# NUStatBioinfo/DegNorm

Hardware: AMD Instinct MI355X
Metric: genes/sec (20k genes x 10 samples, 5 iters) (higher is better)
Workload: dtype f64

## Files before the change

### degnorm_amd/csrc/dn_kernels.hpp

```cpp
#pragma once
#include <hip/hip_runtime.h>
#include <stdint.h>
#include <type_traits>
#include "dn_reduce.hpp"
#include "dn_dpp_ops.hpp"

#ifdef DN_MARKS
#define DN_MARK(name) asm volatile("; DN_MARK " name)
#else
#define DN_MARK(name)
#endif

namespace dn {

constexpr int TRACE_LEN = 48;
constexpr int MAX_BINS = 64;
constexpr int P_MAX = 64;

enum { EXIT_LOW_COV = 0, EXIT_ZERO_SAMPLE = 1, EXIT_MEDIAN = 2, EXIT_NO_LOOP = 3,
       EXIT_REFINED = 4, EXIT_REFINE_FALLBACK = 5, EXIT_NOT_FOUND_FALLBACK = 6 };
enum { LOOP_NATURAL = 0, LOOP_PERFECT = 1, LOOP_VALUE_ERROR = 2, LOOP_ZERO_ROWSUM = 3, LOOP_MIN_BINS = 4,
       LOOP_NOT_ENTERED = 5 };
enum { ST_OK = 0, ST_ARPACK = -1, ST_EMPTY_MIN = -2, ST_VALUE_ERROR = -3,
       ST_NO_CONVERGENCE = -4 };
// ... 1161 lines not shown
        if constexpr (W > 1) {
            dn_sync();
            for (int e = tid; e < NG; e += NT) {
                double tsum = sm.xw[0][e];
#pragma unroll
                for (int ww = 1; ww < W; ww++) tsum += sm.xw[ww][e];
                sm.tot[e] = tsum;
            }
        }
        dn_sync();
    };

    pass(true, 0);
    {
        const double tr = wave_allsum(lane < P ? sm.tot[lane * (lane + 1) / 2 + lane] : 0.0);
        if (!(tr > 0.0)) return ST_ARPACK;
    }
    { const int r = top_eig_rows_lds<P>(sm.tot, uv, vv, theta, maxs); steps += r; noconv = noconv || r > maxs; }
    bool cold_every_solve;
    {
        double um = lane < P ? uv[lane] : 1.0;
#pragma unroll
        for (int o = 32; o >= 1; o >>= 1) um = fmin(um, __shfl_xor(um, o));
        cold_every_solve = __builtin_amdgcn_readfirstlane((int) (um < WARM_START_MIN_COMPONENT)) != 0;
    }
#pragma clang loop unroll(disable)
    for (int t = 0; t < T; t++) {
        pass(false, t);
        int r;
        if (!cold_every_solve) r = top_eig_rows_lds<P>(sm.tot, uv, vv, theta, maxs);
        else {
            unsigned long long todo = P >= 64 ? ~0ull : ((1ull << P) - 1ull);
            double bul = 0.0, bth = -1.0;
            int sum = 0;
            bool capped = false;
            while (todo) {
                const unsigned long long comp = gram_component(sm.tot, __builtin_ctzll(todo), P);
                todo &= ~comp;
                wave_fence();
                uv[lane] = ((comp >> lane) & 1ull) ? 1.0 / sqrt((double) __builtin_popcountll(comp)) : 0.0;
                wave_fence();
                double th = 0.0;
                const int rr = top_eig_rows_lds<P>(sm.tot, uv, vv, th, maxs);
                sum += rr < maxs ? rr : maxs;
                capped = capped || rr > maxs;
                const double ul = uv[lane];
                if (th > bth) { bth = th; bul = ul; }
            }
            wave_fence();
            uv[lane] = bul;
            wave_fence();
            theta = bth > 0.0 ? bth : 0.0;
            r = capped ? maxs + 1 : (sum < maxs ? sum : maxs);
        }
        steps += r; noconv = noconv || r > maxs;
    }
    bcast_rows<P>(lane < P ? uv[lane] : 0.0, u);
    return ST_OK;
}

#ifndef DN_RT_MAX_COLS
#define DN_RT_MAX_COLS 12
#endif
#ifndef DN_RT_MAX_P
#define DN_RT_MAX_P 12
#endif
#ifndef DN_RT_MIN_P
#define DN_RT_MIN_P 2
#endif
#if defined(DN_P) && DN_P >= DN_RT_MIN_P && DN_P <= DN_RT_MAX_P
#define DN_REG_TIER 1
#define DN_KERNEL_WAVES 2
#define DN_RT_CLAIM() asm volatile("" ::: "a255")
#else
#define DN_REG_TIER 0
#define DN_KERNEL_WAVES 1
#define DN_RT_CLAIM()
#endif
#define DN_RAW_MAX_P 12
template <int P> constexpr bool raw_units() { return DN_REG_TIER != 0 && P <= DN_RAW_MAX_P && P < DN_MG_MIN_P; }

template <int IDX> __device__ __forceinline__ int agpr_get1();
template <int IDX> __device__ __forceinline__ void agpr_put1(int v);
#define DN_AGPR_ACCESSORS(N)                                                                                              \
    template <> __device__ __forceinline__ int agpr_get1<N>() { int v; asm volatile("v_accvgpr_read_b32 %0, a" #N : "=v"(v)); return v; } \
    template <> __device__ __forceinline__ void agpr_put1<N>(int v) { asm volatile("v_accvgpr_write_b32 a" #N ", %0" : : "v"(v)); }
#define DN_AGPR_REGS(X) \
    X(0) X(1) X(2) X(3) X(4) X(5) X(6) X(7) X(8) X(9) X(10) X(11) X(12) X(13) X(14) X(15) \
    X(16) X(17) X(18) X(19) X(20) X(21) X(22) X(23) X(24) X(25) X(26) X(27) X(28) X(29) X(30) X(31) \
    X(32) X(33) X(34) X(35) X(36) X(37) X(38) X(39) X(40) X(41) X(42) X(43) X(44) X(45) X(46) X(47) \
    X(48) X(49) X(50) X(51) X(52) X(53) X(54) X(55) X(56) X(57) X(58) X(59) X(60) X(61) X(62) X(63) \
    X(64) X(65) X(66) X(67) X(68) X(69) X(70) X(71) X(72) X(73) X(74) X(75) X(76) X(77) X(78) X(79) \
    X(80) X(81) X(82) X(83) X(84) X(85) X(86) X(87) X(88) X(89) X(90) X(91) X(92) X(93) X(94) X(95) \
    X(96) X(97) X(98) X(99) X(100) X(101) X(102) X(103) X(104) X(105) X(106) X(107) X(108) X(109) X(110) X(111) \
    X(112) X(113) X(114) X(115) X(116) X(117) X(118) X(119) X(120) X(121) X(122) X(123) X(124) X(125) X(126) X(127) \
    X(128) X(129) X(130) X(131) X(132) X(133) X(134) X(135) X(136) X(137) X(138) X(139) X(140) X(141) X(142) X(143) \
    X(144) X(145) X(146) X(147) X(148) X(149) X(150) X(151) X(152) X(153) X(154) X(155) X(156) X(157) X(158) X(159) \
    X(160) X(161) X(162) X(163) X(164) X(165) X(166) X(167) X(168) X(169) X(170) X(171) X(172) X(173) X(174) X(175) \
    X(176) X(177) X(178) X(179) X(180) X(181) X(182) X(183) X(184) X(185) X(186) X(187) X(188) X(189) X(190) X(191) \
    X(192) X(193) X(194) X(195) X(196) X(197) X(198) X(199) X(200) X(201) X(202) X(203) X(204) X(205) X(206) X(207) \
    X(208) X(209) X(210) X(211) X(212) X(213) X(214) X(215) X(216) X(217) X(218) X(219) X(220) X(221) X(222) X(223) \
    X(224) X(225) X(226) X(227) X(228) X(229) X(230) X(231) X(232) X(233) X(234) X(235) X(236) X(237) X(238) X(239) \
    X(240) X(241) X(242) X(243) X(244) X(245) X(246) X(247) X(248) X(249) X(250) X(251) X(252) X(253) X(254) X(255)
DN_AGPR_REGS(DN_AGPR_ACCESSORS)
#undef DN_AGPR_ACCESSORS
#undef DN_AGPR_REGS
template <int IDX> __device__ __forceinline__ double agpr_get()
{
    const int lo = agpr_get1<IDX>(), hi = agpr_get1<IDX + 1>();
    return __hiloint2double(hi, lo);
}
template <int IDX> __device__ __forceinline__ void agpr_put(double v)
{
    agpr_put1<IDX>(__double2loint(v));
    agpr_put1<IDX + 1>(__double2hiint(v));
}

template <int P, int BASE> __device__ __forceinline__ void rt_read(double (&a)[P])
{
    static_for<0, P>([&](auto ic) { constexpr int I = decltype(ic)::value; a[I] = agpr_get<BASE + 2 * I>(); });
}
template <int P, int BASE> __device__ __forceinline__ void rt_write(const double (&a)[P])
{
    static_for<0, P>([&](auto ic) { constexpr int I = decltype(ic)::value; agpr_put<BASE + 2 * I>(a[I]); });
}
template <int P, int BASE> __device__ __forceinline__ void rt_read_counts(double (&xd)[P])
{
    static_for<0, (P + 1) / 2>([&](auto jc) {
        constexpr int J = decltype(jc)::value;
        const unsigned w = (unsigned) agpr_get1<BASE + J>();
        xd[2 * J] = (double) (w & 0xffffu);
        if constexpr (2 * J + 1 < P) xd[2 * J + 1] = (double) (w >> 16);
    });
}
template <int P, int BASE> __device__ __forceinline__ void rt_write_counts(const float (&x)[P])
{
    static_for<0, (P + 1) / 2>([&](auto jc) {
        constexpr int J = decltype(jc)::value;
        unsigned w = (unsigned) x[2 * J];
        if constexpr (2 * J + 1 < P) w |= ((unsigned) x[2 * J + 1]) << 16;
        agpr_put1<BASE + J>((int) w);
    });
}
template <int P, bool X16> constexpr int rt_col_regs() { return 2 * P + (X16 ? (P + 1) / 2 : 0); }
template <int P, bool X16> constexpr int rt_cols()
{
    return (P >= DN_RT_MIN_P && P <= DN_RT_MAX_P) ? (256 / rt_col_regs<P, X16>() < DN_RT_MAX_COLS ? 256 / rt_col_regs<P, X16>() : DN_RT_MAX_COLS) : 0;
}
template <int P> constexpr int rt_regs_used()
{
    return rt_cols<P, true>() * rt_col_regs<P, true>() > rt_cols<P, false>() * rt_col_regs<P, false>()
               ? rt_cols<P, true>() * rt_col_regs<P, true>() : rt_cols<P, false>() * rt_col_regs<P, false>();
}
constexpr int RT_BATCH = 48;
#define DN_RT_SAVE_IDX(r) ((size_t) (r) * NT + DN_TIDX)
template <int N, int NT> __device__ __forceinline__ void rt_save(int *save, int need)
{
    static_for<0, (N + RT_BATCH - 1) / RT_BATCH>([&](auto bc) {
        constexpr int B = decltype(bc)::value * RT_BATCH;
        constexpr int CNT = (N - B) < RT_BATCH ? (N - B) : RT_BATCH;
        if (B < need) {
            int v[CNT];
            static_for<0, CNT>([&](auto ic) { constexpr int I = decltype(ic)::value; v[I] = agpr_get1<B + I>(); });
#pragma unroll
            for (int i = 0; i < CNT; i++) save[DN_RT_SAVE_IDX(B + i)] = v[i];
            asm volatile("" ::: "memory");
        }
    });
}
template <int N, int NT> __device__ __forceinline__ void rt_restore(const int *save, int need)
{
    static_for<0, (N + RT_BATCH - 1) / RT_BATCH>([&](auto bc) {
        constexpr int B = decltype(bc)::value * RT_BATCH;
        constexpr int CNT = (N - B) < RT_BATCH ? (N - B) : RT_BATCH;
        if (B < need) {
            int v[CNT];
#pragma unroll
            for (int i = 0; i < CNT; i++) v[i] = save[DN_RT_SAVE_IDX(B + i)];
            static_for<0, CNT>([&](auto ic) { constexpr int I = decltype(ic)::value; agpr_put1<B + I>(v[I]); });
            asm volatile("" ::: "memory");
        }
    });
}
template <int P, int NT> constexpr size_t rt_save_bytes() { return (size_t) rt_regs_used<P>() * 4 * NT; }

template <int P, int NT, bool X16, bool FULL = false, bool ONCHIP = false, bool SAFE = false>
__device__ __forceinline__ void nmf_body(const float *Fb_, double *Lg_, double *rs_, double *sv_,
                                         int n, int S, int nL, int T, int first_i)
{
    Smem<P, NT> &sm = g_sm;
    double *lam = g_lam + (DN_UNITS > 1 ? (size_t) DN_UNIT * (size_t) nL * (P + (P & 1)) : 0);
    gF_cptr Fb = (gF_cptr) uniform_ptr(Fb_);
    gdouble_ptr Lg = (gdouble_ptr) uniform_ptr(Lg_);
    gdouble_ptr rs = (gdouble_ptr) uniform_ptr(rs_);
    gdouble_ptr sv = (gdouble_ptr) uniform_ptr(sv_);
    n = __builtin_amdgcn_readfirstlane(n);
    S = __builtin_amdgcn_readfirstlane(S);
    nL = __builtin_amdgcn_readfirstlane(nL);
    T = __builtin_amdgcn_readfirstlane(T);
    const bool first = __builtin_amdgcn_readfirstlane(first_i) != 0;
    double inv[P], u[P], theta = 0.0;
    int steps = 0;
    const int maxs = __builtin_amdgcn_readfirstlane(g_gs.max_steps);
    bool noconv = false;
#pragma unroll
    for (int i = 0; i < P; i++) inv[i] = uniform(g_gs.inv[i]);
    long long stamp[4] = {0, 0, 0, 0};
#ifdef DN_STAMP
#define DN_T0() const long long t0_ = __builtin_amdgcn_s_memtime()
#define DN_T1(slot) stamp[slot] += __builtin_amdgcn_s_memtime() - t0_
#else
#define DN_T0()
#define DN_T1(slot) (void) stamp
#endif
    constexpr int NG = P * (P + 1) / 2;
    constexpr int CH_MAX = P <= 15 ? 120 : 90;
    constexpr int SW = (NG + CH_MAX - 1) / CH_MAX;
    constexpr int CH = (NG + SW - 1) / SW;
    constexpr int PS = P + (P & 1);
    const int tid = DN_TIDX;
    constexpr int RT = DN_REG_TIER ? rt_cols<P, X16>() : 0;
    constexpr int CS = rt_col_regs<P, X16>();
    constexpr int NR = RT * NT;
    constexpr bool RAW = raw_units<P>();
    double ud[P], ur[P];
    const int nLe = (n < NR + nL) ? n : NR + nL;
    const int kS0 = NR + nL;
    if constexpr (P >= DN_MG_MIN_P) {
        const int st = mg_core<P, NT>(Fb, Lg, lam, n, nL, T, u, theta, steps, maxs, noconv);
        if (st != ST_OK) { if (tid == 0) g_gs.status = st; dn_sync(); return; }
    } else {
    gram_t G[CH];

#ifdef DN_STAMP
    const long long t_cold0 = __builtin_amdgcn_s_memtime();
#endif
#pragma unroll
    for (int i = 0; i < CH; i++) G[i] = 0.0;
    {
        float xq[P];
        if (tid < n) load_x<P>(Fb, tid, xq);
#pragma clang loop unroll(disable)
        for (int k = tid; k < n; k += NT) {
            double f[P];
#pragma unroll
            for (int i = 0; i < P; i++) f[i] = (double) xq[i] * inv[i];
            load_x<P>(Fb, k + NT < n ? k + NT : k, xq);
            gram_add_range<P, 0, CH>(G, f);
        }
    }
    block_sum_lds<CH, P, NT, gram_t>(G, sm);
    static_for<1, SW>([&](auto qc) {
        constexpr int Q = decltype(qc)::value;
        constexpr int NQ = (NG - Q * CH) < CH ? (NG - Q * CH) : CH;
        gram_t Gq[NQ];
#pragma unroll
        for (int i = 0; i < NQ; i++) Gq[i] = 0.0;
#pragma clang loop unroll(disable)
        for (int k = tid; k < n; k += NT) {
            double f[P];
            load_f<P>(Fb, k, inv, f);
            gram_add_range<P, Q * CH, NQ>(Gq, f);
        }
        block_sum_lds<NQ, P, NT, gram_t, false, Q * CH>(Gq, g_sm);
    });
    {
        double tr = 0.0;
#pragma unroll
        for (int i = 0; i < P; i++) tr += sm.tot[i * (i + 1) / 2 + i];
        if (!(tr > 0.0)) { if (tid == 0) g_gs.status = ST_ARPACK; dn_sync(); return; }
    }
    Solver<P> solver;
    {
        double tr = 0.0;
#pragma unroll
        for (int i = 0; i < P; i++) tr += sm.tot[i * (i + 1) / 2 + i];
        solver.cold(tr, u);
    }
    {
        const int r = SAFE ? solve_by_blocks<P>(solver, sm.tot, Smem<P, NT>::ZSLOT, u, theta, maxs)
                           : solver.run(sm.tot, Smem<P, NT>::ZSLOT, u, theta, T == 0, maxs, true);
        steps += r; noconv = noconv || r > maxs;
    }
    const double c = 1.0 / sqrt((double) T);
    auto pass_u = [&]() {
        if constexpr (RAW) {
            const int k = Solver<P>::row_of_lane() < P ? Solver<P>::row_of_lane() : P - 1;
            const double vt = solver.iterate_of_row() * g_gs.inv[k], vh = solver.iterate_of_row() * g_gs.scl[k];
#pragma unroll
            for (int i = 0; i < P; i++) { ud[i] = Solver<P>::bcast_component(vt, i); ur[i] = Solver<P>::bcast_component(vh, i); }
        } else {
#pragma unroll
            for (int i = 0; i < P; i++) { u[i] = uniform(u[i]); ud[i] = u[i]; ur[i] = u[i]; }
        }
    };
    pass_u();

    static_for<0, RT>([&](auto rc) {
        constexpr int R = decltype(rc)::value;
        const int k = tid + R * NT;
        if (k < n) {
            float xf[P];
            double f[P];
            load_x<P>(Fb, k, xf);
            pass_counts<P, RAW>(xf, inv, f);
            rt_write<P, CS * R>(f);
            if constexpr (X16) rt_write_counts<P, CS * R + 2 * P>(xf);
        }
    });
    for (int k = NR + tid; k < nLe; k += NT) {
        double f[P], a[PS];
        { float xf[P]; load_x<P>(Fb, k, xf); pass_counts<P, RAW>(xf, inv, f); }
#pragma unroll
        for (int i = 0; i < PS; i++) a[i] = i < P ? f[i] : 0.0;
        lds_col_write<PS>(lam + (size_t) (k - NR) * PS, a);
    }
    if constexpr (!ONCHIP) {
        for (int k = kS0 + tid; k < n; k += NT) {
            double f[P];
            { float xf[P]; load_x<P>(Fb, k, xf); pass_counts<P, RAW>(xf, inv, f); }
            spill_col_write<P>(spill_col<P>(Lg, k), f);
        }
    }
#ifdef DN_STAMP
    stamp[3] += __builtin_amdgcn_s_memtime() - t_cold0;
#endif
    constexpr bool G0 = FULL && ONCHIP && SW == 1;
    constexpr bool SQ = Solver<P>::SQUARE && SW == 1 && !SAFE;
#pragma clang loop unroll(disable)
    for (int t = 0; t < T; t++) {
        DN_MARK("iter_begin");
        if constexpr (!G0) {
#pragma unroll
            for (int i = 0; i < CH; i++) G[i] = 0.0;
        }
        DN_MARK("zeroed");
        { DN_T0();
        const int dir = (t & 1) ? -1 : 1;

        auto reg_tier = [&]() {
            if constexpr (RT > 0 && X16) {
                auto column = [&](auto rc) {
                    constexpr int R = decltype(rc)::value;
                    double f[P], a[P];
                    rt_read_counts<P, CS * R + 2 * P>(f);
                    if constexpr (!RAW) {
#pragma unroll
                        for (int i = 0; i < P; i++) f[i] *= inv[i];
                    }
                    rt_read<P, CS * R>(a);
                    col_update<P>(f, a, ud, ur, c);
                    if constexpr (G0 && R == 0) gram_set_range<P, 0, CH>(G, a); else gram_add_range<P, 0, CH>(G, a);
                    rt_write<P, CS * R>(a);
                };
                if constexpr (FULL) {
                    static_for<0, RT>([&](auto rc) { column(rc); __builtin_amdgcn_sched_barrier(0); });
                } else {
                    static_for<0, RT>([&](auto rc) {
                        constexpr int R = decltype(rc)::value;
                        if (tid + R * NT < n) column(rc);
                    });
                }
            } else if constexpr (RT > 0) {
                float xq[P];
                if (tid < n) load_x<P>(Fb, tid, xq);
                static_for<0, RT>([&](auto rc) {
                    constexpr int R = decltype(rc)::value;
                    const int k = tid + R * NT;
                    if (k < n) {
                        double f[P], a[P];
                        pass_counts<P, RAW>(xq, inv, f);
                        if constexpr (R + 1 < RT) load_x<P>(Fb, k + NT < n ? k + NT : k, xq);
                        rt_read<P, CS * R>(a);
                        col_update<P>(f, a, ud, ur, c);
                        gram_add_range<P, 0, CH>(G, a);
                        rt_write<P, CS * R>(a);
                    }
                });
            }
        };
        auto lds_tier = [&]() {
            const int first = NR + tid;
            const int cnt = first < nLe ? (nLe - first + NT - 1) / NT : 0;
            const int step = dir * NT;
            int k = dir > 0 ? first : first + (cnt - 1) * NT;
            float xq[P];
            if (cnt > 0) load_x<P>(Fb, k, xq);
#pragma clang loop unroll(disable)
            for (int j = 0; j < cnt; j++, k += step) {
                double f[P], a[PS];
                lds_col_read<PS>(lam + (size_t) (k - NR) * PS, a);
                pass_counts<P, RAW>(xq, inv, f);
                load_x<P>(Fb, j + 1 < cnt ? k + step : k, xq);
                double aa[P];
#pragma unroll
                for (int i = 0; i < P; i++) aa[i] = a[i];
                col_update<P>(f, aa, ud, ur, c);
                gram_add_range<P, 0, CH>(G, aa);
#pragma unroll
                for (int i = 0; i < P; i++) a[i] = aa[i];
                lds_col_write<PS>(lam + (size_t) (k - NR) * PS, a);
            }
        };
        auto spill_tier = [&]() {
            if constexpr (ONCHIP) return;
            int tq = tid;
            asm volatile("" : "+v"(tq));
            const int first = kS0 + tq;
            if (first >= n) return;
            const int step = dir * NT;
            const int last = first + (n - 1 - first) / NT * NT;
            int k = dir > 0 ? first : last;
            const int kend = dir > 0 ? last : first;
            float xn[P];
            double an[P];
            load_x<P>(Fb, k, xn);
            spill_col_read<P>(spill_col<P>(Lg, k), an);
            bool more;
#pragma clang loop unroll(disable)
            do {
                double f[P], a[P];
                pass_counts<P, RAW>(xn, inv, f);
#pragma unroll
                for (int i = 0; i < P; i++) a[i] = an[i];
                const int kn = dir > 0 ? min(k + step, kend) : max(k + step, kend);
                load_x<P>(Fb, kn, xn);
                spill_col_read<P>(spill_col<P>(Lg, kn), an);
                col_update<P>(f, a, ud, ur, c);
                gram_add_range<P, 0, CH>(G, a);
                spill_col_write<P>(spill_col<P>(Lg, k), a);
                more = k != kend;
                k += step;
            } while (more);
        };
#if defined(DN_STAMP) && defined(DN_EXP_TIER)
#define DN_TIER(id, call) do { if (DN_EXP_TIER == id) { const long long tt_ = __builtin_amdgcn_s_memtime(); call; stamp[0] += __builtin_amdgcn_s_memtime() - tt_; } else { call; } } while (0)
#else
#define DN_TIER(id, call) call
#endif
        if constexpr (G0) { DN_MARK("reg_tier"); DN_TIER(1, reg_tier()); DN_MARK("lds_tier"); DN_TIER(2, lds_tier()); }
        else if (dir > 0) { DN_MARK("reg_tier"); DN_TIER(1, reg_tier()); DN_MARK("lds_tier"); DN_TIER(2, lds_tier()); DN_MARK("spill_tier"); DN_TIER(3, spill_tier()); }
        else { DN_MARK("spill_tier_b"); DN_TIER(3, spill_tier()); DN_MARK("lds_tier_b"); DN_TIER(2, lds_tier()); DN_MARK("reg_tier_b"); DN_TIER(1, reg_tier()); }
        DN_MARK("pass_end");
#if !(defined(DN_STAMP) && defined(DN_EXP_TIER))
        DN_T1(0);
#endif
        }
        { DN_T0(); block_sum_lds<CH, P, NT, gram_t, Solver<P>::SHIFTED, 0, RAW, SQ>(G, sm, solver.shift(), solver.scale(), t & 1); DN_T1(1); }
        DN_MARK("reduced");
        static_for<1, SW>([&](auto qc) {
            constexpr int Q = decltype(qc)::value;
            constexpr int NQ = (NG - Q * CH) < CH ? (NG - Q * CH) : CH;
            gram_t Gq[NQ];
#pragma unroll
            for (int i = 0; i < NQ; i++) Gq[i] = 0.0;
            static_assert(SW == 1 || RT == 0, "the later sweeps do not read the register tier");
#pragma clang loop unroll(disable)
            for (int k = NR + tid; k < nLe; k += NT) {
                double a[PS], aa[P];
                lds_col_read<PS>(lam + (size_t) (k - NR) * PS, a);
#pragma unroll
                for (int i = 0; i < P; i++) aa[i] = a[i];
                gram_add_range<P, Q * CH, NQ>(Gq, aa);
            }
#pragma clang loop unroll(disable)
            for (int k = kS0 + tid; k < n; k += NT) {
                double aa[P];
                spill_col_read<P>(spill_col<P>(Lg, k), aa);
                gram_add_range<P, Q * CH, NQ>(Gq, aa);
            }
            block_sum_lds<NQ, P, NT, gram_t, Solver<P>::SHIFTED, Q * CH>(Gq, g_sm, solver.shift());
        });
        { DN_T0();
        double u_unused[P];
        double (&us_)[P] = RAW ? u_unused : u;
        const int r = SAFE ? solve_by_blocks<P>(solver, sm.tot, Smem<P, NT>::ZSLOT, us_, theta, maxs)
                           : solver.template run<SQ>(sm.tot, Smem<P, NT>::ZSLOT, us_, theta, t == T - 1, maxs, false,
                                                     sm.sq + wave_id() * Smem<P, NT>::SQ_LEN);
        steps += r; noconv = noconv || r > maxs;
        pass_u();
        DN_MARK("solved");
        DN_T1(2);
        }
    }
    if constexpr (SQ && NT > 64) dn_sync();
    if constexpr (RAW) {
#pragma unroll
        for (int i = 0; i < P; i++) u[i] = Solver<P>::bcast_component(solver.iterate_of_row(), i);
    }
    }

#ifdef DN_STAMP
    const long long t_fin0 = __builtin_amdgcn_s_memtime();
#endif
    double invf[P];
#pragma unroll
    for (int i = 0; i < P; i++) invf[i] = RAW ? uniform(g_gs.inv[i]) : inv[i];
    double acc[2 * P + 1];
#pragma unroll
    for (int i = 0; i < 2 * P + 1; i++) acc[i] = 0.0;
    auto fin = [&](int k, const double (&f)[P], const double (&l_)[P]) {
        double s, r, l0[P];
#pragma unroll
        for (int i = 0; i < P; i++) l0[i] = RAW ? l_[i] * invf[i] : l_[i];
        col_final<P>(f, l0, u, first, acc, s, r);
        rs[k] = r;
        if (first) sv[k] = s;
    };
    static_for<0, RT>([&](auto rc) {
        constexpr int R = decltype(rc)::value;
        const int k = tid + R * NT;
        if (k < n) {
            double f[P], l[P];
            if constexpr (X16) {
                rt_read_counts<P, CS * R + 2 * P>(f);
#pragma unroll
                for (int i = 0; i < P; i++) f[i] *= invf[i];
            } else load_f<P>(Fb, k, invf, f);
            rt_read<P, CS * R>(l);
            fin(k, f, l);
        }
    });
    float xqf[P];
    if (NR + tid < n) load_x<P>(Fb, NR + tid, xqf);
#pragma clang loop unroll(disable)
    for (int k = NR + tid; k < n; k += NT) {
        double f[P], l[P];
#pragma unroll
        for (int i = 0; i < P; i++) f[i] = (double) xqf[i] * invf[i];
        load_x<P>(Fb, k + NT < n ? k + NT : k, xqf);
        if (k < nLe) {
            double al[PS];
            lds_col_read<PS>(lam + (size_t) (k - NR) * PS, al);
#pragma unroll
            for (int i = 0; i < P; i++) l[i] = al[i];
        } else spill_col_read<P>(spill_col<P>(Lg, k), l);
        fin(k, f, l);
    }
    block_sum_lds<2 * P + 1, P, NT, double>(acc, sm);
    for (int e = tid; e < 2 * P + 1; e += NT) g_gs.sums[e] = sm.tot[e];
    if (tid == 0) {
#pragma unroll
        for (int i = 0; i < P; i++) g_gs.u[i] = u[i];
        g_gs.theta = theta;
        g_gs.steps += steps;
        g_gs.status = noconv ? ST_NO_CONVERGENCE : ST_OK;
#ifdef DN_STAMP
        g_gs.stamp[0] += stamp[0]; g_gs.stamp[1] += stamp[1]; g_gs.stamp[2] += stamp[2];
        g_gs.stamp[4] += __builtin_amdgcn_s_memtime() - t_fin0; g_gs.stamp[5] += stamp[3];
#endif
    }
    dn_sync();
}

template <int P, int NT, bool SAFE = false>
__device__ __attribute__((noinline)) void nmf_call(const float *Fb_, double *Lg_, double *rs_, double *sv_, double *rtsave_,
                                                   int n, int S, int nL, int T, int first_i, int x16_i)
{
    constexpr int NSAVE = DN_REG_TIER ? rt_regs_used<P>() : 0;
    int *rtsave = reinterpret_cast<int *>(uniform_ptr(rtsave_));
#ifdef DN_STAMP
    const long long t_call0 = __builtin_amdgcn_s_memtime();
#endif
    const int n_u = __builtin_amdgcn_readfirstlane(n);
    const int need = DN_REG_TIER ? ((n_u + NT - 1) / NT) * rt_col_regs<P, true>() : 0;
    rt_save<NSAVE, NT>(rtsave, need);
    if constexpr (SAFE) {
        nmf_body<P, NT, false, false, false, true>(Fb_, Lg_, rs_, sv_, n, S, nL, T, first_i);
    } else if (DN_REG_TIER && __builtin_amdgcn_readfirstlane(x16_i) != 0) {
        constexpr bool X = DN_REG_TIER != 0;
        const int nL_u = __builtin_amdgcn_readfirstlane(nL);
        if (X && n_u >= rt_cols<P, X>() * NT && n_u <= rt_cols<P, X>() * NT + nL_u)
            nmf_body<P, NT, X, X, X>(Fb_, Lg_, rs_, sv_, n, S, nL, T, first_i);
        else if (X && n_u >= rt_cols<P, X>() * NT) nmf_body<P, NT, X, X>(Fb_, Lg_, rs_, sv_, n, S, nL, T, first_i);
        else nmf_body<P, NT, X, false>(Fb_, Lg_, rs_, sv_, n, S, nL, T, first_i);
    } else nmf_body<P, NT, false>(Fb_, Lg_, rs_, sv_, n, S, nL, T, first_i);
    rt_restore<NSAVE, NT>(rtsave, need);
#ifdef DN_STAMP
    if (DN_TIDX == 0) g_gs.stamp[3] += __builtin_amdgcn_s_memtime() - t_call0;
#endif
}


template <int P> __device__ __forceinline__ double lds_max(const double *v)
{ double m = v[0];
#pragma unroll
  for (int i = 1; i < P; i++) { const double t = v[i]; m = t > m ? t : m; } return m; }
template <int P> __device__ __forceinline__ double lds_min(const double *v)
{ double m = v[0];
#pragma unroll
  for (int i = 1; i < P; i++) { const double t = v[i]; m = t < m ? t : m; } return m; }

template <int P, int NT>
__global__ __launch_bounds__(NT * DN_UNITS, DN_KERNEL_WAVES) void k_baseline(IterArgs A)
{
    constexpr int W = NT / 64;
    Smem<P, NT> &sm = g_sm;
    GeneState<P> &gs = g_gs;
    const int tid = DN_TIDX, lane = lane_id(), w = wave_id();
    const int S = A.S;
    const int nL = A.lds_cols;
    char *slot = A.ws + ((size_t) blockIdx.x * DN_UNITS + DN_UNIT) * A.slot_bytes;
    float *Fs = reinterpret_cast<float *>(slot);
    float *Fb = Fs + (size_t) P * S;
    double *Lg = reinterpret_cast<double *>(Fb + (size_t) P * S);
    double *sv = Lg + (size_t) (P + (P & 1)) * S;
    double *rs = sv + S;
    double *rtsave = rs + 2 * (size_t) S;
    DN_RT_CLAIM();
    if (tid < P) { gs.inv[tid] = A.inv_scale[tid]; gs.scl[tid] = 1.0 / A.inv_scale[tid]; }
    if (tid == 0) gs.max_steps = A.max_steps > 0 ? A.max_steps : EIG_MAX_STEPS_DEFAULT;
    if constexpr (P <= 16) { for (int t = tid; t < W * Smem<P, NT>::SQ_LEN; t += NT) sm.sq[t] = 0.0; }
    for (int t = tid; t < Smem<P, NT>::NX; t += NT) {
        bool diag = false;
        int ra = 0, rb = 0;
#pragma unroll
        for (int i = 0; i < P; i++) {
            diag = diag || (t == i * (i + 1) / 2 + i);
            if (t >= i * (i + 1) / 2) { ra = i; rb = t - i * (i + 1) / 2; }
        }
        if constexpr (P <= 16) sm.sqi[t] = (t < P * (P + 1) / 2) ? (ra * Smem<P, NT>::SQ_STR + rb) | ((rb * Smem<P, NT>::SQ_STR + ra) << 16) : 0;
        if constexpr (raw_units<P>())
            sm.dsel[t] = (t < P * (P + 1) / 2) ? (diag ? -1.0 : 1.0) * A.inv_scale[ra] * A.inv_scale[rb < P ? rb : 0] : 0.0;
        else sm.dsel[t] = diag ? 1.0 : 0.0;
        if (t == Smem<P, NT>::ZSLOT) sm.tot[t] = 0.0;
    }

    for (;;) {
        if (tid == 0) sm.gene = atomicAdd(A.counter, 1);
        dn_sync();
        const int q = sm.gene;
        dn_sync();
        if (q >= A.n_genes) break;
        const int g = A.order[q];
        const int L = A.glen[g];
        const float *x = A.cov + A.goff[g];

        int n0 = 0, n_calls = 0, n_drops = 0, exit_code = EXIT_LOW_COV, loop_reason = LOOP_NOT_ENTERED;
        int status = ST_OK, flag = 0, emode = EM_INPUT;
        long long sum_cols = 0;
#ifdef DN_STAMP
        const long long t_gene0 = __builtin_amdgcn_s_memtime();
        long long t_ret = 0, t_book = 0;
#endif
        int32_t *tr = A.trace + (size_t) g * TRACE_LEN;
        if (tid < P) { gs.rho[tid] = 0.0; gs.K[tid] = 0.0; gs.us[tid] = 0.0; }
        if (tid == 0) { gs.steps = 0; gs.stamp[0] = gs.stamp[1] = gs.stamp[2] = gs.stamp[3] = gs.stamp[4] = gs.stamp[5] = 0; }

        double thr;
        int x16;
        {
            const float *rmx = A.rowmax + (size_t) g * P;
            double gmax = (double) rmx[0] / A.scale[0];
#pragma unroll
            for (int i = 1; i < P; i++) { const double v = (double) rmx[i] / A.scale[i]; gmax = v > gmax ? v : gmax; }
            thr = 0.1 * gmax;
            x16 = A.x16[g];
        }

        const int rate = A.rate;
        const long long ds0 = (rate > 1 && A.ds_start) ? A.ds_start[g] : -1;
        const int M = ds0 >= 0 ? (ds0 < L ? (int) ((L - 1 - ds0) / rate) + 1 : 0) : L;
        const int seg = ((M + W - 1) / W + 63) & ~63;
        const int jb = w * seg, je = (jb + seg < M) ? jb + seg : M;

        {
            double sumF[P];
#pragma unroll
            for (int i = 0; i < P; i++) sumF[i] = 0.0;
            int base = 0;
            for (int pass = 0; pass < 2; pass++) {
                int run = 0;
                for (int c = jb; c < je; c += 64) {
                    const int m = c + lane;
                    bool hi = false;
                    float xv[P];
                    double f[P];
                    if (m < je) {
                        const long long j = ds0 >= 0 ? ds0 + (long long) m * rate : (long long) m;
                        double cm = 0.0;
#pragma unroll
                        for (int i = 0; i < P; i++) { xv[i] = x[(size_t) i * L + j]; f[i] = (double) xv[i] / A.scale[i]; cm = f[i] > cm ? f[i] : cm; }
                        hi = cm > thr;
                    }
                    const unsigned long long mask = __ballot(hi);
                    if (pass == 1 && hi) {
                        const int pos = base + run + __popcll(mask & ((1ull << lane) - 1ull));
#pragma unroll
                        for (int i = 0; i < P; i++) {
                            Fs[(size_t) i * S + pos] = xv[i];
                            Fb[(size_t) pos * P + i] = xv[i];
                            sumF[i] += f[i];
                        }
                    }
                    run += __popcll(mask);
                }
                if (pass == 0) {
                    if (lane == 0) sm.cnt[w] = run;
                    dn_sync();
                    n0 = 0;
#pragma unroll
                    for (int ww = 0; ww < W; ww++) { if (ww < w) base += sm.cnt[ww]; n0 += sm.cnt[ww]; }
                    dn_sync();
                    if (n0 < A.min_hc) break;
                }
            }
            if (n0 >= A.min_hc) {
                block_sum<P, P, NT>(sumF, sm);
                if (tid == 0) {
#pragma unroll
                    for (int i = 0; i < P; i++) gs.sumF[i] = sumF[i];
                }
            }
            dn_sync();
        }

#ifdef DN_STAMP
        const long long t_scan1 = __builtin_amdgcn_s_memtime();
#endif
        int n = n0;
        if (n0 >= A.min_hc) {
            if (!(lds_min<P>(gs.sumF) > 0.0)) exit_code = EXIT_ZERO_SAMPLE;
            else {
                const double min_gene_len = fmax(2.0, ceil(200.0 * (1.0 / (double) rate)));
                const double min_bins = ceil((double) A.bins * 0.2);
                int csize = 1, n_bins = 0;
                bool first = true, in_loop = false;
                for (;;) {
#ifdef DN_STAMP
                    if (t_ret != 0) t_book += __builtin_amdgcn_s_memtime() - t_ret;
#endif
                    nmf_call<P, NT>(Fb, Lg, rs, sv, rtsave, n, S, nL, A.T, first ? 1 : 0, x16);
                    if constexpr (P < DN_MG_MIN_P) {
                        const int st_call = __builtin_amdgcn_readfirstlane(gs.status);
                        bool unsafe = st_call == ST_NO_CONVERGENCE;
                        if (st_call == ST_OK) {
#pragma unroll
                            for (int i = 0; i < P; i++)
                                unsafe = unsafe || (gs.u[i] < WARM_START_MIN_COMPONENT && gs.sums[1 + P + i] > 0.0);
                        }
                        if (__builtin_amdgcn_readfirstlane((int) unsafe) != 0) {
                            dn_sync();
                            nmf_call<P, NT, true>(Fb, Lg, rs, sv, rtsave, n, S, nL, A.T, first ? 1 : 0, x16);
                        }
                    }
#ifdef DN_STAMP
                    t_ret = __builtin_amdgcn_s_memtime();
#endif
                    if (gs.status != ST_OK) { status = gs.status; break; }
                    const double *u = gs.u, *sums = gs.sums;
                    const double theta = gs.theta;
                    n_calls++; sum_cols += n;
                    if (first) {
                        if (tid == 0) {
                            const double sig = sqrt(theta);
                            gs.sig0 = sig;
#pragma unroll
                            for (int i = 0; i < P; i++) {
                                gs.us[i] = u[i];
                                gs.K[i] = u[i] * sig;
                                gs.rho[i] = 1.0 - sums[1 + P + i] / (u[i] * sums[0] + 1.0);
                                gs.rho_fb[i] = 1.0 - gs.sumF[i] / (sums[1 + i] + 1.0);
                            }
                        }
                        dn_sync();
                        double med;
                        {
                            double om[P];
#pragma unroll
                            for (int i = 0; i < P; i++) om[i] = 1.0 - gs.rho[i];
                            med = median_of<P>(om);
                        }
                        if (med > 1.0) { exit_code = EXIT_MEDIAN; break; }
                        emode = (n0 < L) ? EM_EXPAND : EM_RAW;
                        exit_code = EXIT_NO_LOOP;
                        if (!((double) n0 >= min_gene_len && lds_min<P>(gs.rho) <= 0.2 && !A.skip)) break;
                        in_loop = true;
                        csize = (n0 + A.bins - 1) / A.bins;
                        n_bins = (n0 + csize - 1) / csize;
                        if (tid < n_bins) sm.alive[tid] = tid;
                        dn_sync();
                        first = false;
                    } else {
                        bool zero_row = false;
#pragma unroll
                        for (int i = 0; i < P; i++) zero_row = zero_row || (sums[1 + P + i] == 0.0);
                        if (tid == 0) {
                            const double sg = sqrt(theta);
#pragma unroll
                            for (int i = 0; i < P; i++) {
                                gs.K[i] = u[i] * sg;
                                if (!zero_row) gs.rho[i] = 1.0 - sums[1 + P + i] / (sums[1 + i] + 1.0);
                            }
                        }
                        dn_sync();
                        if (zero_row) { loop_reason = LOOP_ZERO_ROWSUM; break; }
                        if ((double) n_bins <= min_bins || (double) n < min_gene_len) { loop_reason = LOOP_MIN_BINS; break; }
                    }
                    if (!(lds_max<P>(gs.rho) > 0.1)) break;
                    flag = 1;
                    loop_reason = LOOP_NATURAL;
                    for (int b = w; b < n_bins; b += W) {
                        const int kb = b * csize, ke = (kb + csize < n) ? kb + csize : n;
                        double part = 0.0;
                        for (int k = kb + lane; k < ke; k += 4 * 64) {
                            double v[4];
#pragma unroll
                            for (int c = 0; c < 4; c++) v[c] = (k + 64 * c < ke) ? rs[k + 64 * c] : 0.0;
#pragma unroll
                            for (int c = 0; c < 4; c++) if (k + 64 * c < ke) part += v[c];
                        }
                        part = wave_sum1(part);
                        if (lane == 0) sm.ss[b] = part / (double) (ke - kb);
                    }
                    dn_sync();
                    double best = -INFINITY; int drop = 0;
                    for (int b = 0; b < n_bins; b++) { const double v = sm.ss[b]; if (v > best) { best = v; drop = b; } }
                    dn_sync();
                    if (best == 0.0) { loop_reason = LOOP_PERFECT; break; }
                    const int kb = drop * csize;
                    const int dlen = ((kb + csize < n) ? kb + csize : n) - kb;
                    if (tid == 0) {
                        for (int b = drop; b < n_bins - 1; b++) sm.alive[b] = sm.alive[b + 1];
                        if (n_drops < 32) tr[8 + n_drops] = drop;
                    }
                    n_bins--;
                    n -= dlen;
                    n_drops++;
                    dn_sync();
                    for (int k0 = kb + tid; k0 < n; k0 += 4 * NT) {
                        float v[4][P];
#pragma unroll
                        for (int c = 0; c < 4; c++) {
                            const int k = (k0 + c * NT < n) ? k0 + c * NT : k0;
                            const int a = k / csize;
                            const int ko = sm.alive[a] * csize + (k - a * csize);
#pragma unroll
                            for (int i = 0; i < P; i++) v[c][i] = Fs[(size_t) i * S + ko];
                        }
#pragma unroll
                        for (int c = 0; c < 4; c++) {
                            if (k0 + c * NT < n) {
#pragma unroll
                                for (int i = 0; i < P; i++) Fb[(size_t) (k0 + c * NT) * P + i] = v[c][i];
                            }
                        }
                    }
                    dn_sync();
                    if (n < 2) { loop_reason = LOOP_VALUE_ERROR; break; }
                }

                if (in_loop && status == ST_OK) {
                    bool fallback = false;
                    if (lds_max<P>(gs.rho) < 0.2) {
                        double K[P];
#pragma unroll
                        for (int i = 0; i < P; i++) K[i] = gs.K[i];
                        status = fix_k<P>(K);
                        if (status == ST_OK) {
                            double se[1] = {0.0};
                            for (int k = tid; k < n0; k += NT) {
                                double m = -INFINITY;
#pragma unroll
                                for (int i = 0; i < P; i++) {
                                    const double qv = ((double) Fs[(size_t) i * S + k] * gs.inv[i]) / K[i];
                                    m = qv > m ? qv : m;
                                }
                                se[0] += m;
                            }
                            block_sum<1, P, NT>(se, sm);
                            double rmax = -INFINITY;
#pragma unroll
                            for (int i = 0; i < P; i++) {
                                const double r = 1.0 - gs.sumF[i] / (K[i] * se[0] + 1.0);
                                rmax = r > rmax ? r : rmax;
                            }
                            dn_sync();
                            if (rmax > 0.9) { fallback = true; exit_code = EXIT_REFINE_FALLBACK; }
                            else {
                                exit_code = EXIT_REFINED; emode = (n0 < L) ? EM_EXPAND : EM_REFINED;
                                if (tid == 0) {
#pragma unroll
                                    for (int i = 0; i < P; i++) { gs.K[i] = K[i]; gs.rho[i] = 1.0 - gs.sumF[i] / (K[i] * se[0] + 1.0); }
                                }
                            }
                        }
                    } else { fallback = true; exit_code = EXIT_NOT_FOUND_FALLBACK; }
                    if (fallback && status == ST_OK) {
                        if (tid == 0) {
#pragma unroll
                            for (int i = 0; i < P; i++) { gs.K[i] = gs.us[i] * gs.sig0; gs.rho[i] = gs.rho_fb[i]; }
                        }
                        emode = (n0 < L) ? EM_EXPAND : EM_CLAMPED;
                    }
                    dn_sync();
                }
                if (status == ST_OK && exit_code >= EXIT_NO_LOOP && n0 < L) {
                    double K[P];
#pragma unroll
                    for (int i = 0; i < P; i++) K[i] = gs.K[i];
                    status = fix_k<P>(K);
                    dn_sync();
                    if (tid == 0) {
#pragma unroll
                        for (int i = 0; i < P; i++) gs.K[i] = K[i];
                    }
                }
            }
        }
        dn_sync();

        const bool zero_out = (status != ST_OK) || exit_code <= EXIT_MEDIAN;
        if (zero_out) { emode = EM_INPUT; if (status != ST_OK) flag = 0; }

        if (tid == 0) {
#pragma unroll
            for (int i = 0; i < P; i++) {
                A.rho[(size_t) g * P + i] = zero_out ? 0.0 : gs.rho[i];
                A.kfin[(size_t) g * P + i] = (emode == EM_CLAMPED || emode == EM_RAW) ? gs.us[i] : gs.K[i];
            }
            A.flags[g] = flag;
            A.emode[g] = emode;
            tr[0] = n0; tr[1] = n_calls; tr[2] = (int32_t) sum_cols; tr[3] = exit_code; tr[4] = loop_reason;
            tr[5] = n_drops; tr[6] = status; tr[7] = gs.steps;
#ifdef DN_STAMP
            tr[40] = (int32_t) (gs.stamp[0] >> 10); tr[41] = (int32_t) (gs.stamp[1] >> 10); tr[42] = (int32_t) (gs.stamp[2] >> 10);
            tr[44] = (int32_t) (gs.stamp[3] >> 10); tr[45] = (int32_t) (gs.stamp[4] >> 10); tr[46] = (int32_t) (gs.stamp[5] >> 10);
            tr[43] = (int32_t) ((__builtin_amdgcn_s_memtime() - t_gene0) >> 10);
            tr[47] = (int32_t) ((t_scan1 - t_gene0) >> 10);
            tr[39] = (int32_t) (t_book >> 10);
            tr[38] = (int32_t) ((t_ret != 0 ? __builtin_amdgcn_s_memtime() - t_ret : 0) >> 10);
#endif
        }
        if (A.want_est && (emode == EM_CLAMPED || emode == EM_RAW)) {
            double *dst = A.svec + A.svoff[g];
            for (int k = tid; k < n0; k += NT) dst[k] = sv[k];
        }
        dn_sync();
    }
}

template <int P, int NT>
__global__ __launch_bounds__(NT) void k_ratio_svd(InitArgs A)
{
    constexpr int NG = P * (P + 1) / 2;
    Smem<P, NT> &sm = g_sm;
    const int tid = DN_TIDX;
    for (;;) {
        if (tid == 0) sm.gene = atomicAdd(A.counter, 1);
        dn_sync();
        const int q = sm.gene;
        dn_sync();
        if (q >= A.n_genes) break;
        const int g = A.order[q];
        const int L = A.glen[g];
        const float *x = A.cov + A.goff[g];
        int status = ST_OK;
        double acc[2 * P];
#pragma unroll
        for (int i = 0; i < 2 * P; i++) acc[i] = 0.0;
        if (L < 2) status = ST_VALUE_ERROR;
        else {
            double G[NG];
#pragma unroll
            for (int i = 0; i < NG; i++) G[i] = 0.0;
            for (int j = tid; j < L; j += NT) {
// ... 112 lines not shown
```

Before: 15440.

## Software-pipeline LDS tier loop two columns per iteration with prefetched reads

Rewrites the LDS-resident column loop to handle two columns per iteration. The next column's LDS read is issued before the current column's Gram accumulation and write-back, so LDS latency can overlap with compute. Scheduling barriers pin the interleaving. Separately, the non-convergence flag is packed into a high bit of the step counter to save a register. Risks include higher register pressure and subtle edge handling for odd counts and direction.

Result: no change. 15500 (median of 6 runs) (+0.4%).

```diff
diff --git a/degnorm_amd/csrc/dn_kernels.hpp b/degnorm_amd/csrc/dn_kernels.hpp
--- a/degnorm_amd/csrc/dn_kernels.hpp
+++ b/degnorm_amd/csrc/dn_kernels.hpp
@@ -1388,6 +1388,7 @@
     int steps = 0;
     const int maxs = __builtin_amdgcn_readfirstlane(g_gs.max_steps);
     bool noconv = false;
+    constexpr int NOCONV_BIT = 1 << 30;
 #pragma unroll
     for (int i = 0; i < P; i++) inv[i] = uniform(g_gs.inv[i]);
     long long stamp[4] = {0, 0, 0, 0};
@@ -1465,7 +1466,7 @@
     {
         const int r = SAFE ? solve_by_blocks<P>(solver, sm.tot, Smem<P, NT>::ZSLOT, u, theta, maxs)
                            : solver.run(sm.tot, Smem<P, NT>::ZSLOT, u, theta, T == 0, maxs, true);
-        steps += r; noconv = noconv || r > maxs;
+        steps = (steps + r) | (r > maxs ? NOCONV_BIT : 0);
     }
     const double c = 1.0 / sqrt((double) T);
     auto pass_u = [&]() {
@@ -1565,27 +1566,72 @@
             }
         };
         auto lds_tier = [&]() {
-            const int first = NR + tid;
-            const int cnt = first < nLe ? (nLe - first + NT - 1) / NT : 0;
+            int tq;
+            asm volatile("v_mov_b32 %0, %1" : "=v"(tq) : "v"(tid));
+            const int first = NR + tq;
+            if (first >= nLe) return;
             const int step = dir * NT;
-            int k = dir > 0 ? first : first + (cnt - 1) * NT;
+            const int last = first + (nLe - 1 - first) / NT * NT;
+            int k = dir > 0 ? first : last;
+            const int kend = dir > 0 ? last : first;
+            double *const pend = lam + (size_t) (kend - NR) * PS;
+            auto next_k = [&](int kk) {
+                if constexpr (G0) return kk != kend ? kk + step : kk;
+                else return dir > 0 ? min(kk + step, kend) : max(kk + step, kend);
+            };
+            auto next_p = [&](double *pp, int kk) {
+                double *const pn = pp + step * PS;
+                if constexpr (G0) return kk != kend ? pn : pp;
+                else return dir > 0 ? (pn < pend ? pn : pend) : (pn > pend ? pn : pend);
+            };
+            double *pa = lam + (size_t) (k - NR) * PS;
             float xq[P];
-            if (cnt > 0) load_x<P>(Fb, k, xq);
+            double a1[PS];
+            load_x<P>(Fb, k, xq);
+            lds_col_read<PS>(pa, a1);
+            bool more;
 #pragma clang loop unroll(disable)
-            for (int j = 0; j < cnt; j++, k += step) {
-                double f[P], a[PS];
-                lds_col_read<PS>(lam + (size_t) (k - NR) * PS, a);
-                pass_counts<P, RAW>(xq, inv, f);
-                load_x<P>(Fb, j + 1 < cnt ? k + step : k, xq);
-                double aa[P];
-#pragma unroll
-                for (int i = 0; i < P; i++) aa[i] = a[i];
-                col_update<P>(f, aa, ud, ur, c);
+            do {
+                double f1[P], a2[PS], aa[P];
+                pass_counts<P, RAW>(xq, inv, f1);
+                const int k0 = k;
+                const int kb = next_k(k);
+                double *const pb = next_p(pa, k);
+                load_x<P>(Fb, kb, xq);
+#pragma unroll
+                for (int i = 0; i < P; i++) aa[i] = a1[i];
+                col_update<P>(f1, aa, ud, ur, c);
+                __builtin_amdgcn_sched_barrier(0);
+                lds_col_read<PS>(pb, a2);
+                __builtin_amdgcn_sched_barrier(0);
                 gram_add_range<P, 0, CH>(G, aa);
-#pragma unroll
-                for (int i = 0; i < P; i++) a[i] = aa[i];
-                lds_col_write<PS>(lam + (size_t) (k - NR) * PS, a);
-            }
+                __builtin_amdgcn_sched_barrier(0);
+#pragma unroll
+                for (int i = 0; i < P; i++) a1[i] = aa[i];
+                lds_col_write<PS>(pa, a1);
+                __builtin_amdgcn_sched_barrier(0);
+                double f2[P], bb[P];
+                pass_counts<P, RAW>(xq, inv, f2);
+                more = kb != kend;
+                k = next_k(kb);
+                pa = next_p(pb, kb);
+                load_x<P>(Fb, k, xq);
+#pragma unroll
+                for (int i = 0; i < P; i++) bb[i] = a2[i];
+                col_update<P>(f2, bb, ud, ur, c);
+#pragma unroll
+                for (int i = 0; i < P; i++) asm volatile("" : "+v"(bb[i]));
+                __builtin_amdgcn_sched_barrier(0);
+                lds_col_read<PS>(pa, a1);
+                __builtin_amdgcn_sched_barrier(0);
+                if (k0 != kend) {
+                    gram_add_range<P, 0, CH>(G, bb);
+                    __builtin_amdgcn_sched_barrier(0);
+#pragma unroll
+                    for (int i = 0; i < P; i++) a2[i] = bb[i];
+                    lds_col_write<PS>(pb, a2);
+                }
+            } while (more);
         };
         auto spill_tier = [&]() {
             if constexpr (ONCHIP) return;
@@ -1662,12 +1708,14 @@
         const int r = SAFE ? solve_by_blocks<P>(solver, sm.tot, Smem<P, NT>::ZSLOT, us_, theta, maxs)
                            : solver.template run<SQ>(sm.tot, Smem<P, NT>::ZSLOT, us_, theta, t == T - 1, maxs, false,
                                                      sm.sq + wave_id() * Smem<P, NT>::SQ_LEN);
-        steps += r; noconv = noconv || r > maxs;
+        steps = (steps + r) | (r > maxs ? NOCONV_BIT : 0);
         pass_u();
         DN_MARK("solved");
         DN_T1(2);
         }
     }
+    noconv = (steps & NOCONV_BIT) != 0;
+    steps &= NOCONV_BIT - 1;
     if constexpr (SQ && NT > 64) dn_sync();
     if constexpr (RAW) {
 #pragma unroll
```

## Vectorize register-tier save/restore and batch loads in init, finalize and bin scan

Applied to the files above, without the earlier changes.

Register-tier save/restore now moves data with 16-byte vector global accesses in a layout grouped by four, and uses a larger batch when the tier is big. The initial fill of the register, LDS and spill tiers issues several column loads before doing any compute. The finalize loop is split into an LDS part and a spill part, and the spill part prefetches the next spill column. The bin-mean scan loads the first chunk of four bins at once before reducing them. The aim is more memory-level parallelism and fewer load/store instructions, at the cost of extra register pressure and a changed save-buffer layout that must stay consistent between save and restore.

Result: no change. 15440 before, 15540 after (median of 6 runs) (+0.7%).

```diff
diff --git a/degnorm_amd/csrc/dn_kernels.hpp b/degnorm_amd/csrc/dn_kernels.hpp
--- a/degnorm_amd/csrc/dn_kernels.hpp
+++ b/degnorm_amd/csrc/dn_kernels.hpp
@@ -1337,31 +1337,63 @@
     return rt_cols<P, true>() * rt_col_regs<P, true>() > rt_cols<P, false>() * rt_col_regs<P, false>()
                ? rt_cols<P, true>() * rt_col_regs<P, true>() : rt_cols<P, false>() * rt_col_regs<P, false>();
 }
-constexpr int RT_BATCH = 48;
-#define DN_RT_SAVE_IDX(r) ((size_t) (r) * NT + DN_TIDX)
+template <int N> constexpr int rt_batch() { return N > 128 ? 128 : 48; }
+typedef int dn_i4 __attribute__((ext_vector_type(4)));
+typedef int dn_i2 __attribute__((ext_vector_type(2)));
 template <int N, int NT> __device__ __forceinline__ void rt_save(int *save, int need)
 {
+    typedef dn_i4 __attribute__((address_space(1))) *gi4_ptr;
+    typedef dn_i2 __attribute__((address_space(1))) *gi2_ptr;
+    typedef int __attribute__((address_space(1))) *gi_ptr;
+    constexpr int RT_BATCH = rt_batch<N>();
+    static_assert(RT_BATCH % 4 == 0, "a batch is a whole number of 16-byte groups");
+    const int tid = DN_TIDX;
     static_for<0, (N + RT_BATCH - 1) / RT_BATCH>([&](auto bc) {
         constexpr int B = decltype(bc)::value * RT_BATCH;
         constexpr int CNT = (N - B) < RT_BATCH ? (N - B) : RT_BATCH;
+        constexpr int G = CNT / 4, TAIL = CNT % 4;
         if (B < need) {
             int v[CNT];
             static_for<0, CNT>([&](auto ic) { constexpr int I = decltype(ic)::value; v[I] = agpr_get1<B + I>(); });
-#pragma unroll
-            for (int i = 0; i < CNT; i++) save[DN_RT_SAVE_IDX(B + i)] = v[i];
+            gi4_ptr s4 = (gi4_ptr) save + (size_t) (B / 4) * NT + tid;
+#pragma unroll
+            for (int g = 0; g < G; g++) s4[(size_t) g * NT] = dn_i4{v[4 * g], v[4 * g + 1], v[4 * g + 2], v[4 * g + 3]};
+            if constexpr (TAIL == 2) *((gi2_ptr) ((gi_ptr) save + (size_t) (B + 4 * G) * NT) + tid) = dn_i2{v[4 * G], v[4 * G + 1]};
+            else if constexpr (TAIL != 0) {
+#pragma unroll
+                for (int i = 0; i < TAIL; i++) ((gi_ptr) save)[(size_t) (B + 4 * G) * NT + (size_t) tid * TAIL + i] = v[4 * G + i];
+            }
             asm volatile("" ::: "memory");
         }
     });
 }
 template <int N, int NT> __device__ __forceinline__ void rt_restore(const int *save, int need)
 {
+    typedef const dn_i4 __attribute__((address_space(1))) *gi4_cptr;
+    typedef const dn_i2 __attribute__((address_space(1))) *gi2_cptr;
+    typedef const int __attribute__((address_space(1))) *gi_cptr;
+    constexpr int RT_BATCH = rt_batch<N>();
+    static_assert(RT_BATCH % 4 == 0, "a batch is a whole number of 16-byte groups");
+    const int tid = DN_TIDX;
     static_for<0, (N + RT_BATCH - 1) / RT_BATCH>([&](auto bc) {
         constexpr int B = decltype(bc)::value * RT_BATCH;
         constexpr int CNT = (N - B) < RT_BATCH ? (N - B) : RT_BATCH;
+        constexpr int G = CNT / 4, TAIL = CNT % 4;
         if (B < need) {
             int v[CNT];
-#pragma unroll
-            for (int i = 0; i < CNT; i++) v[i] = save[DN_RT_SAVE_IDX(B + i)];
+            gi4_cptr s4 = (gi4_cptr) save + (size_t) (B / 4) * NT + tid;
+#pragma unroll
+            for (int g = 0; g < G; g++) {
+                const dn_i4 q = s4[(size_t) g * NT];
+                v[4 * g] = q.x; v[4 * g + 1] = q.y; v[4 * g + 2] = q.z; v[4 * g + 3] = q.w;
+            }
+            if constexpr (TAIL == 2) {
+                const dn_i2 q = *((gi2_cptr) ((gi_cptr) save + (size_t) (B + 4 * G) * NT) + tid);
+                v[4 * G] = q.x; v[4 * G + 1] = q.y;
+            } else if constexpr (TAIL != 0) {
+#pragma unroll
+                for (int i = 0; i < TAIL; i++) v[4 * G + i] = ((gi_cptr) save)[(size_t) (B + 4 * G) * NT + (size_t) tid * TAIL + i];
+            }
             static_for<0, CNT>([&](auto ic) { constexpr int I = decltype(ic)::value; agpr_put1<B + I>(v[I]); });
             asm volatile("" ::: "memory");
         }
@@ -1481,30 +1513,52 @@
     };
     pass_u();
 
-    static_for<0, RT>([&](auto rc) {
-        constexpr int R = decltype(rc)::value;
-        const int k = tid + R * NT;
-        if (k < n) {
-            float xf[P];
-            double f[P];
-            load_x<P>(Fb, k, xf);
-            pass_counts<P, RAW>(xf, inv, f);
-            rt_write<P, CS * R>(f);
-            if constexpr (X16) rt_write_counts<P, CS * R + 2 * P>(xf);
-        }
-    });
-    for (int k = NR + tid; k < nLe; k += NT) {
-        double f[P], a[PS];
-        { float xf[P]; load_x<P>(Fb, k, xf); pass_counts<P, RAW>(xf, inv, f); }
-#pragma unroll
-        for (int i = 0; i < PS; i++) a[i] = i < P ? f[i] : 0.0;
-        lds_col_write<PS>(lam + (size_t) (k - NR) * PS, a);
-    }
-    if constexpr (!ONCHIP) {
-        for (int k = kS0 + tid; k < n; k += NT) {
-            double f[P];
-            { float xf[P]; load_x<P>(Fb, k, xf); pass_counts<P, RAW>(xf, inv, f); }
-            spill_col_write<P>(spill_col<P>(Lg, k), f);
+    {
+        int tc = tid;
+        asm volatile("" : "+v"(tc));
+        if constexpr (RT > 0) {
+            float xr[RT][P];
+            static_for<0, RT>([&](auto rc) {
+                constexpr int R = decltype(rc)::value;
+                const int k = tc + R * NT;
+                load_x<P>(Fb, FULL || k < n ? k : n - 1, xr[R]);
+            });
+            static_for<0, RT>([&](auto rc) {
+                constexpr int R = decltype(rc)::value;
+                if (FULL || tc + R * NT < n) {
+                    double f[P];
+                    pass_counts<P, RAW>(xr[R], inv, f);
+                    rt_write<P, CS * R>(f);
+                    if constexpr (X16) rt_write_counts<P, CS * R + 2 * P>(xr[R]);
+                }
+            });
+        }
+        constexpr int COLD_U = 4;
+        auto init_tier = [&](int first, int end, auto &&put) {
+            if (first < end) {
+                const int last = first + (end - 1 - first) / NT * NT;
+#pragma clang loop unroll(disable)
+                for (int k0 = first; k0 <= last; k0 += COLD_U * NT) {
+                    float xf[COLD_U][P];
+#pragma unroll
+                    for (int j = 0; j < COLD_U; j++) load_x<P>(Fb, min(k0 + j * NT, last), xf[j]);
+#pragma unroll
+                    for (int j = 0; j < COLD_U; j++) {
+                        double f[P];
+                        pass_counts<P, RAW>(xf[j], inv, f);
+                        put(min(k0 + j * NT, last), f);
+                    }
+                }
+            }
+        };
+        init_tier(NR + tc, nLe, [&](int k, const double (&f)[P]) {
+            double a[PS];
+#pragma unroll
+            for (int i = 0; i < PS; i++) a[i] = i < P ? f[i < P ? i : 0] : 0.0;
+            lds_col_write<PS>(lam + (size_t) (k - NR) * PS, a);
+        });
+        if constexpr (!ONCHIP) {
+            init_tier(kS0 + tc, n, [&](int k, const double (&f)[P]) { spill_col_write<P>(spill_col<P>(Lg, k), f); });
         }
     }
 #ifdef DN_STAMP
@@ -1706,21 +1760,43 @@
             fin(k, f, l);
         }
     });
-    float xqf[P];
-    if (NR + tid < n) load_x<P>(Fb, NR + tid, xqf);
+    {
+        constexpr bool SPF = P <= 16;
+        int tf = tid;
+        asm volatile("" : "+v"(tf));
+        int k = NR + tf;
+        float xqf[P];
+        if (k < n) load_x<P>(Fb, k, xqf);
 #pragma clang loop unroll(disable)
-    for (int k = NR + tid; k < n; k += NT) {
-        double f[P], l[P];
-#pragma unroll
-        for (int i = 0; i < P; i++) f[i] = (double) xqf[i] * invf[i];
-        load_x<P>(Fb, k + NT < n ? k + NT : k, xqf);
-        if (k < nLe) {
-            double al[PS];
+        for (; k < nLe; k += NT) {
+            double f[P], l[P], al[PS];
+#pragma unroll
+            for (int i = 0; i < P; i++) f[i] = (double) xqf[i] * invf[i];
+            load_x<P>(Fb, k + NT < n ? k + NT : k, xqf);
             lds_col_read<PS>(lam + (size_t) (k - NR) * PS, al);
 #pragma unroll
             for (int i = 0; i < P; i++) l[i] = al[i];
-        } else spill_col_read<P>(spill_col<P>(Lg, k), l);
-        fin(k, f, l);
+            fin(k, f, l);
+        }
+        if (k < n) {
+            const int last = k + (n - 1 - k) / NT * NT;
+            double lq[SPF ? P : 1];
+            if constexpr (SPF) spill_col_read<P>(spill_col<P>(Lg, k), lq);
+#pragma clang loop unroll(disable)
+            for (; k <= last; k += NT) {
+                double f[P], l[P];
+#pragma unroll
+                for (int i = 0; i < P; i++) f[i] = (double) xqf[i] * invf[i];
+                const int kn = min(k + NT, last);
+                load_x<P>(Fb, kn, xqf);
+                if constexpr (SPF) {
+#pragma unroll
+                    for (int i = 0; i < P; i++) l[i] = lq[i];
+                    spill_col_read<P>(spill_col<P>(Lg, kn), lq);
+                } else spill_col_read<P>(spill_col<P>(Lg, k), l);
+                fin(k, f, l);
+            }
+        }
     }
     block_sum_lds<2 * P + 1, P, NT, double>(acc, sm);
     for (int e = tid; e < 2 * P + 1; e += NT) g_gs.sums[e] = sm.tot[e];
@@ -1985,18 +2061,34 @@
                     if (!(lds_max<P>(gs.rho) > 0.1)) break;
                     flag = 1;
                     loop_reason = LOOP_NATURAL;
-                    for (int b = w; b < n_bins; b += W) {
-                        const int kb = b * csize, ke = (kb + csize < n) ? kb + csize : n;
-                        double part = 0.0;
-                        for (int k = kb + lane; k < ke; k += 4 * 64) {
-                            double v[4];
-#pragma unroll
-                            for (int c = 0; c < 4; c++) v[c] = (k + 64 * c < ke) ? rs[k + 64 * c] : 0.0;
-#pragma unroll
-                            for (int c = 0; c < 4; c++) if (k + 64 * c < ke) part += v[c];
+                    constexpr int BIF = 4;
+                    for (int b0 = w; b0 < n_bins; b0 += BIF * W) {
+                        double v[BIF][4];
+#pragma unroll
+                        for (int j = 0; j < BIF; j++) {
+                            const int b = b0 + j * W;
+                            const int kb = b * csize, ke = (kb + csize < n) ? kb + csize : n, k = kb + lane;
+#pragma unroll
+                            for (int c = 0; c < 4; c++) v[j][c] = (b < n_bins && k + 64 * c < ke) ? rs[k + 64 * c] : 0.0;
                         }
-                        part = wave_sum1(part);
-                        if (lane == 0) sm.ss[b] = part / (double) (ke - kb);
+#pragma unroll
+                        for (int j = 0; j < BIF; j++) {
+                            const int b = b0 + j * W;
+                            if (b >= n_bins) break;
+                            const int kb = b * csize, ke = (kb + csize < n) ? kb + csize : n;
+                            double part = 0.0;
+#pragma unroll
+                            for (int c = 0; c < 4; c++) if (kb + lane + 64 * c < ke) part += v[j][c];
+                            for (int k = kb + lane + 4 * 64; k < ke; k += 4 * 64) {
+                                double u4[4];
+#pragma unroll
+                                for (int c = 0; c < 4; c++) u4[c] = (k + 64 * c < ke) ? rs[k + 64 * c] : 0.0;
+#pragma unroll
+                                for (int c = 0; c < 4; c++) if (k + 64 * c < ke) part += u4[c];
+                            }
+                            part = wave_sum1(part);
+                            if (lane == 0) sm.ss[b] = part / (double) (ke - kb);
+                        }
                     }
                     dn_sync();
                     double best = -INFINITY; int drop = 0;
```
